# yf26/Hands-On-Point-Cloud-Processing

Measured on AMD Instinct MI355X. Metric: M correspondences/sec + ICP iter/sec, 120k-pt KITTI pair, 1/2/4/8 MI355X, higher is better.
Workload: dtype f32

## Files before the change

hands-on-point-cloud-processing_amd/__init__.py:

```python
from __future__ import annotations

import ctypes as C
import os
import weakref

import numpy as np

_HERE = os.path.dirname(os.path.abspath(__file__))
LIB_PATH = os.environ.get("PCR_LIB_PATH") or os.path.join(_HERE, "libpcr_hip.so")
INCLUDE_DIR = os.path.join(os.path.dirname(_HERE), "include")

PCR_SOA, PCR_AOS3, PCR_AOS4, PCR_AOS6 = 0, 1, 2, 6
PCR_FPS_F32, PCR_FPS_F64 = 0, 1
PCR_KMEANS_PY, PCR_KMEANS_CPP = 0, 1
PCR_EMPTY_CLUSTER = 1
PCR_SPECTRAL_DUPLICATE, PCR_SPECTRAL_COMPLEX, PCR_SPECTRAL_NOT_CONVERGED, PCR_SPECTRAL_FEW_SEEDS = 2, 3, 4, 5
ERRORS = {0: "ok", -1: "bad argument", -2: "HIP error", -3: "out of memory", -4: "bad state",
          -5: "RCCL/collective error", -6: "no correspondence kept"}

_lib = None


class PcrError(RuntimeError):
    pass
# ... 77 lines not shown
    _fields_ = [("kind", C.c_int32), ("reserved0", C.c_uint32), ("beta1", C.c_double), ("beta2", C.c_double), ("eps", C.c_double), ("weight_decay", C.c_double),
                ("momentum", C.c_double), ("dampening", C.c_double), ("reserved", C.c_double * 4)]


class OptimInfo(C.Structure):
    _fields_ = [("desc", OptimDesc), ("step", C.c_uint64), ("state_bytes", C.c_uint64), ("attached", C.c_uint32), ("n_ranges", C.c_uint32)]


OPTIM_ADAM, OPTIM_SGD = 1, 2

ALLREDUCE_FN = C.CFUNCTYPE(C.c_int, C.c_void_p, C.POINTER(C.c_double), C.c_int)

ABI_SYMBOLS = [
    "pcr_device_count", "pcr_ctx_create", "pcr_ctx_destroy", "pcr_ctx_sync", "pcr_ctx_last_error", "pcr_version", "pcr_ctx_device_info",
    "pcr_cloud_create", "pcr_cloud_clone", "pcr_cloud_assign", "pcr_cloud_read", "pcr_cloud_size", "pcr_cloud_destroy",
    "pcr_nn1_f32", "pcr_nn1_f32_async", "pcr_nn1_fetch", "pcr_transform_f32", "pcr_kabsch_sums", "pcr_kabsch_solve", "pcr_kabsch_grid_exponent", "pcr_kabsch_limbs_to_sums",
    "pcr_icp_p2p_f32", "pcr_icp_last_chain", "pcr_icp_last_snapshots", "pcr_icp_replica_members", "pcr_icp_move_route", "pcr_icp_solve_route", "pcr_icp_solve_in_search_auto", "pcr_s3_walk_visits", "pcr_plane_count_f64", "pcr_plane_mask_f64", "pcr_knn_f64", "pcr_radius_f64",
    "pcr_comm_unique_id", "pcr_comm_init_rccl", "pcr_comm_init_callback", "pcr_comm_destroy", "pcr_comm_selftest", "pcr_shard_range",
    "pcr_prof_reset", "pcr_prof_get", "pcr_prof_get_each", "pcr_tune_set",
    "pcr_grid_stats", "pcr_nn1_stats", "pcr_selftest_mfma_bf16", "pcr_selftest_mfma_f16", "pcr_selftest_mfma_bf16_v2", "pcr_selftest_mfma_f16_v2", "pcr_selftest_sign_f16", "pcr_selftest_sphere_f16", "pcr_ctx_mfma_check", "pcr_voxel_filter_f32", "pcr_iss_keypoints_f32", "pcr_icp_p2plane_f32", "pcr_cloud_knn_f64", "pcr_normals_knn_f64", "pcr_cloud_pca_f64", "pcr_fast_eigen3x3", "pcr_ground_seeds_f64", "pcr_ground_detection_f64",
    "pcr_nn1_desc_f32", "pcr_match_union_f32", "pcr_match_inter_f32", "pcr_ransac_sample_quads", "pcr_consensus_count_f32", "pcr_ransac_global_f32", "pcr_db64_create", "pcr_db64_destroy", "pcr_db64_size", "pcr_db64_knn", "pcr_db64_radius",
    "pcr_ctx_trim", "pcr_ctx_parked_bytes", "pcr_cloud_shard_spatial", "pcr_cloud_global_index", "pcr_cloud_sort_for_target", "pcr_nn1_f32_loop",
    "pcr_db64_radius_rows", "pcr_rows_destroy", "pcr_rows_info", "pcr_rows_row_ptr", "pcr_rows_fetch", "pcr_rows_reduce", "pcr_rows_moments",
    "pcr_dbscan_f32", "pcr_statistical_outlier_f32", "pcr_fpfh33_f32", "pcr_harris3d_f32", "pcr_voxel_grid_normals_f32", "pcr_normal_space_sample_f32",
    "pcr_fps_f32", "pcr_ball_query_f32", "pcr_group_points_f32", "pcr_objects_from_labels_f32", "pcr_points_in_boxes_f64", "pcr_label_aabb_f32",
    "pcr_pn2_model_create", "pcr_pn2_model_destroy", "pcr_pn2_model_info", "pcr_sa_mlp_max_f32", "pcr_pn2_forward_f32",
    "pcr_pn2_msg_model_create", "pcr_pn2_msg_model_info", "pcr_ball_query_multi_f32", "pcr_sa_msg_mlp_max_f32",
    "pcr_pn1_model_create", "pcr_pn1_model_info", "pcr_pointwise_chain_max_f32", "pcr_pointnet_forward_f32",
    "pcr_pn2_trainer_create", "pcr_pn2_trainer_destroy", "pcr_pn2_trainer_info", "pcr_pn2_trainer_set_weights", "pcr_pn2_trainer_get_weights", "pcr_pn2_train_grad_f32",
    "pcr_pn1_trainer_create", "pcr_pointnet_train_grad_f32",
    "pcr_pn2_msg_trainer_create", "pcr_pn2_msg_trainer_info",
# ... 32 lines not shown
    L.pcr_cloud_size.restype = sz
    L.pcr_cloud_size.argtypes = [vp]
    L.pcr_cloud_destroy.argtypes = [vp, vp]
    L.pcr_nn1_f32.argtypes = [vp, vp, vp, vp, vp]
    L.pcr_nn1_f32_async.argtypes = [vp, vp, vp]
    L.pcr_nn1_fetch.argtypes = [vp, sz, vp, vp]
    L.pcr_ctx_trim.argtypes = [vp]
    L.pcr_cloud_shard_spatial.argtypes = [vp, vp, vp, C.c_int, C.c_int, C.c_int, C.POINTER(vp)]
    L.pcr_cloud_global_index.argtypes = [vp, vp, vp]
    L.pcr_ctx_parked_bytes.argtypes = [vp, C.POINTER(C.c_uint64)]
    L.pcr_cloud_sort_for_target.argtypes = [vp, vp, vp, vp]
    L.pcr_nn1_f32_loop.argtypes = [vp, vp, vp, C.c_float]
    L.pcr_transform_f32.argtypes = [vp, vp, vp]
    L.pcr_kabsch_sums.argtypes = [vp, vp, vp, C.c_float, vp, C.POINTER(C.c_int64), C.POINTER(C.c_float)]
    L.pcr_kabsch_solve.argtypes = [vp, vp, vp]
    L.pcr_kabsch_grid_exponent.argtypes = [C.c_float, C.c_float]
    L.pcr_kabsch_limbs_to_sums.argtypes = [vp, C.c_int, vp]
    L.pcr_icp_p2p_f32.argtypes = [vp, vp, vp, vp, C.POINTER(IcpParams), vp, C.POINTER(IcpStats)]
    L.pcr_icp_last_chain.argtypes = [vp]
    L.pcr_icp_last_snapshots.argtypes = [vp]
    L.pcr_icp_replica_members.argtypes = [C.c_uint32, C.c_uint32]
    L.pcr_icp_replica_members.restype = C.c_uint32
    L.pcr_icp_move_route.argtypes = [C.c_uint64, C.c_uint64, C.c_int] + [C.c_int64] * 7
    L.pcr_icp_solve_route.argtypes = [C.c_uint64, C.c_uint64, C.c_int] + [C.c_int64] * 8
    L.pcr_icp_solve_in_search_auto.argtypes = []
    L.pcr_icp_solve_in_search_auto.restype = C.c_uint64
    L.pcr_s3_walk_visits.argtypes = [C.c_uint32, vp, vp, C.c_uint32, vp, sz, C.POINTER(sz)]
    L.pcr_plane_count_f64.argtypes = [vp, vp, vp, sz, C.c_double, vp]
    L.pcr_plane_mask_f64.argtypes = [vp, vp, vp, C.c_double, vp, C.POINTER(C.c_int64)]
    L.pcr_knn_f64.argtypes = [vp, vp, sz, vp, sz, C.c_int, vp, vp]
# ... 207 lines not shown


def spectral_select_k(eigenvalues) -> int:
    e = np.ascontiguousarray(eigenvalues, np.float64)
    return int(lib().pcr_spectral_select_k(e.ctypes.data, e.shape[0]))


def kabsch_solve(sums):
    s = np.ascontiguousarray(sums, np.float64)
    R = np.zeros(9, np.float32)
    t = np.zeros(3, np.float32)
    rc = lib().pcr_kabsch_solve(s.ctypes.data, R.ctypes.data, t.ctypes.data)
    return rc, R.reshape(3, 3), t


class Cloud:

    def __init__(self, ctx: "Context", handle):
        self.ctx = ctx
        self.h = handle
        ctx._handles.add(self)

    def __del__(self):
        try:
            self.free()
        except Exception:
            pass

    def __len__(self):
        return int(lib().pcr_cloud_size(self.h))
# ... 1325 lines not shown
                                             qd.ctypes.data, qd.shape[0], thr, R.ctypes.data, tv.ctypes.data, C.byref(best), C.byref(win),
                                             counts.ctypes.data))
        return win.value, R.reshape(3, 3), tv, best.value, counts[: qd.shape[0]]

    def transform(self, cloud: Cloud, T):
        T = np.ascontiguousarray(T, np.float32).reshape(16)
        self._ck(lib().pcr_transform_f32(self.h, cloud.h, T.ctypes.data))

    def kabsch_sums(self, tgt: Cloud, src: Cloud, max_corr: float):
        sums = np.zeros(16, np.float64)
        last = C.c_int64()
        d2 = C.c_float()
        self._ck(lib().pcr_kabsch_sums(self.h, tgt.h, src.h, max_corr, sums.ctypes.data, C.byref(last), C.byref(d2)))
        return sums, last.value, d2.value

    def icp_point2point(self, src: Cloud, tgt: Cloud, init_T=None, max_corr=1.0, max_iter=20, eps=1e-8):
        T0 = np.eye(4, dtype=np.float32) if init_T is None else np.ascontiguousarray(init_T, np.float32)
        out = np.zeros(16, np.float32)
        prm = IcpParams(max_corr, max_iter, eps)
        st = IcpStats()
        self._ck(lib().pcr_icp_p2p_f32(self.h, src.h, tgt.h, T0.ctypes.data, C.byref(prm), out.ctypes.data, C.byref(st)))
        stats = {f: getattr(st, f) for f, _ in IcpStats._fields_ if f != "reserved"}
        return out.reshape(4, 4), stats

    def icp_last_chain(self) -> int:
        return int(lib().pcr_icp_last_chain(self.h))

    def icp_last_snapshots(self) -> int:
        return int(lib().pcr_icp_last_snapshots(self.h))

# ... 74 lines not shown
```

hands-on-point-cloud-processing_amd/csrc/api.cpp:

```cpp
#include "pcr_internal.hpp"
#include "numerics.hpp"

#include <cmath>
#include <limits>
#include <new>

namespace pcr {

int fail(pcr_ctx* ctx, int code, const char* what, hipError_t e)
{
    if (ctx) {
        ctx->err = what ? what : "";
        if (e != hipSuccess) {
            ctx->err += ": ";
            ctx->err += hipGetErrorString(e);
        }
    }
    return code;
}

int ensure_keys(pcr_ctx* ctx, size_t n)
{
    if (n <= ctx->keys_cap) return PCR_OK;
    if (ctx->keys) PCR_HIP(ctx, hipFree(ctx->keys));
// ... 516 lines not shown

int pcr_kabsch_limbs_to_sums(double row[55], int e, double sums[16])
{
    if (!row || !sums) return PCR_ERR_ARG;
    num::limbs_normalize_row(row);
    num::limbs_to_sums(row, e, sums);
    return PCR_OK;
}

int pcr_kabsch_solve(const double sums[16], float R[9], float t[3])
{
    if (!sums || !R || !t) return PCR_ERR_ARG;
    return kabsch_solve(sums, R, t);
}

int pcr_prof_reset(pcr_ctx* ctx)
{
    if (!ctx) return PCR_ERR_ARG;
    PCR_HIP(ctx, hipStreamSynchronize(ctx->stream));
    prof_flush(ctx);
    ctx->prof.clear();
    return PCR_OK;
}

int pcr_prof_get(pcr_ctx* ctx, const char* kernel, uint64_t* launches, double* total_ms)
{
    if (!ctx || !kernel) return PCR_ERR_ARG;
    PCR_HIP(ctx, hipStreamSynchronize(ctx->stream));
    prof_flush(ctx);
    auto it = ctx->prof.find(kernel);
// ... 228 lines not shown
```

hands-on-point-cloud-processing_amd/csrc/icp_finish.hpp:

```cpp
#pragma once

#include "pcr_internal.hpp"
#include "numerics.hpp"

#include <cstddef>

#pragma clang fp contract(off)

namespace pcr {

constexpr int KB_NL = num::KB_NL;
constexpr int KB_ROW = 58;
constexpr int KB_NLC = 40;

__device__ __forceinline__ void row_to_out18(int k, const double (&row)[KB_ROW], int e, double* out)
{
    if (k < 6) out[k] = num::limbs_value(row + 3 * k, 2, e - 2 * num::KB_W);
    else if (k < 15) out[k] = num::limbs_value(row + 18 + 4 * (k - 6), 3, 2 * e - 3 * num::KB_W);
    else if (k == 15) out[15] = row[54];
    else if (k == 16) {
        const unsigned long long lk = (unsigned long long)__double_as_longlong(row[55]);
        out[16] = row[54] > 0.0 ? (double)(uint32_t)(lk >> 32) : -1.0;
        out[17] = row[54] > 0.0 ? (double)__uint_as_float((uint32_t)(lk & 0xFFFFFFFFull)) : 0.0;
        out[18] = row[56];
// ... 65 lines not shown
    } else if (k == 15) {
        row[54] = (double)s_acc[0][KB_NLC - 1];
    } else if (k == 16) {
        row[55] = __longlong_as_double(s_acc[0][KB_NLC + 1]);
        row[56] = s_acc[0][KB_NLC] != 0 ? 1.0 : 0.0;
        row[57] = 0.0;
    }
}

__device__ __forceinline__ void fin_wave_sync()
{
    __builtin_amdgcn_fence(__ATOMIC_ACQ_REL, "wavefront");
    __builtin_amdgcn_wave_barrier();
}

struct IcpFinishLds {
    long long acc[ACC_R][ACC_W];
    double row[KB_ROW];
    double o18[19];
    IcpState st;
#ifdef PCR_SV_PROF
    unsigned long long pt_replicas;
#endif
};

constexpr int FIN_ACC_PER_LANE = ACC_R * ACC_W / 64;
static_assert(ACC_R * ACC_W % 64 == 0, "a wave reads the replicas in whole rounds");
struct IcpFinishLoads {
    uint32_t stw;
    long long acc[FIN_ACC_PER_LANE];
// ... 17 lines not shown
        fin_wave_sync();
        return false;
    }
#pragma unroll
    for (int i = 0; i < FIN_ACC_PER_LANE; i++) (&F.acc[0][0])[l + 64 * i] = Q.acc[i];
    fin_wave_sync();
#ifdef PCR_SV_PROF
    if (l == 0) F.pt_replicas = __builtin_amdgcn_s_memrealtime();
#endif
    if (l < KB_NLC + 2) acc_fold_column(F.acc, l);
    fin_wave_sync();
    acc_to_row(F.acc, l, F.row);
    fin_wave_sync();
    row_to_out18(l, F.row, e, F.o18);
    fin_wave_sync();
    if (l == 0) icp_state_step(&F.st, F.o18, F.o18[16] >= 0.0, (float)F.o18[17], F.o18[18] != 0.0);
    fin_wave_sync();
    return true;
}

__device__ __forceinline__ void finish_publish(int l, bool stepped, const IcpFinishLds& F, IcpState* st_out, double* out, IcpSnapSlot* snap, unsigned long long seq)
{
    static_assert(offsetof(IcpSnapSlot, state) == 0, "a snapshot's words, and behind them its sequence number");
    if (stepped && l < 19) out[l] = F.o18[l];
    if (l < ST_WORDS) reinterpret_cast<uint32_t*>(st_out)[l] = reinterpret_cast<const uint32_t*>(&F.st)[l];
    if (!snap) return;
    if (l < ST_WORDS) reinterpret_cast<uint32_t*>(&snap->state)[l] = reinterpret_cast<const uint32_t*>(&F.st)[l];
    fin_wave_sync();
    if (l == 0) __hip_atomic_store(&snap->seq, seq, __ATOMIC_RELEASE, __HIP_MEMORY_SCOPE_SYSTEM);
}

}
// ... 1 lines not shown
```

hands-on-point-cloud-processing_amd/csrc/kabsch.hip:

```cpp
#include "grid_common.hpp"
#include "icp_finish.hpp"
#include "numerics.hpp"

#include <algorithm>
#include <cmath>
#include <cstddef>

#pragma clang fp contract(off)

namespace pcr {

constexpr int KB_BLOCK = 256;
constexpr int KB_NV = 16;
constexpr int KB_MAX_BLOCKS = 8192;
static_assert(KB_ROW * KB_MAX_BLOCKS == 8192 * 58, "api.cpp sizes ctx->partials as 8192 x 58 doubles");

__device__ __forceinline__ double wave_sum(double v)
{
#pragma unroll
    for (int off = 32; off > 0; off >>= 1) v += __shfl_down(v, off, 64);
    return v;
}

__device__ __forceinline__ unsigned long long wave_max_u64(unsigned long long v)
// ... 341 lines not shown

__global__ __launch_bounds__(KF_BLOCK) void icp_update_kernel(const double* __restrict__ partials, uint32_t n_blocks, int e, IcpState* st,
                                                              double* __restrict__ out)
{
    __shared__ double red[KF_GROUPS][64];
    __shared__ double row[KB_ROW];
    __shared__ double o18[19];
    __shared__ IcpState s_st;
    icp_state_stage(st, &s_st);
    if (s_st.stop) return;
    if (s_st.stop_after_transform) { if (threadIdx.x == 0) st->stop = 1; return; }
    reduce_rows(partials, n_blocks, red, row);
    row_to_out18(row, e, o18);
    __syncthreads();
    if (threadIdx.x < 19) out[threadIdx.x] = o18[threadIdx.x];
    if (threadIdx.x == 0) {
        icp_state_step(&s_st, o18, o18[16] >= 0.0, (float)o18[17], o18[18] != 0.0);
        *st = s_st;
    }
}

struct SeedArgs {
    const float* tx; const float* ty; const float* tz;
    unsigned long long* keys;
    uint32_t nt;
};

__device__ __forceinline__ void seed_next_search(const SeedArgs& sd, uint32_t i, uint32_t n, float x, float y, float z)
{
    if (i >= n) return;
    const uint32_t j = (uint32_t)(sd.keys[i] & 0xFFFFFFFFull);
    unsigned long long key = ~0ull;
    if (j < sd.nt) {
// ... 23 lines not shown
        for (int u = 0; u < 4; u++)
            if (4 * i + u < n) sk[u] = sd.keys[4 * i + u];
#pragma unroll
        for (int u = 0; u < 4; u++) {
            const uint32_t j = (uint32_t)(sk[u] & 0xFFFFFFFFull);
            if (j < sd.nt) { sq[u][0] = sd.tx[j]; sq[u][1] = sd.ty[j]; sq[u][2] = sd.tz[j]; }
        }
    }
    icp_state_stage(st_in, &s_st);
    const int phase = s_st.stop ? 0 : (s_st.stop_after_transform ? 1 : 2);
    if (phase == 2) {
        reduce_rows(partials, n_blocks, red, row);
        row_to_out18(row, e, o18);
        __syncthreads();
        if (blockIdx.x == 0 && threadIdx.x < 19) out[threadIdx.x] = o18[threadIdx.x];
        if (threadIdx.x == 0) icp_state_step(&s_st, o18, o18[16] >= 0.0, (float)o18[17], o18[18] != 0.0);
    } else if (phase == 1) {
        if (threadIdx.x == 0) s_st.stop = 1;
    }
    __syncthreads();
    if (blockIdx.x == 0 && threadIdx.x == 0) *st_out = s_st;
    if (s_st.stop || !mine) return;
    const float r0 = s_st.Rd[0], r1 = s_st.Rd[1], r2 = s_st.Rd[2], r3 = s_st.Rd[3], r4 = s_st.Rd[4], r5 = s_st.Rd[5],
                r6 = s_st.Rd[6], r7 = s_st.Rd[7], r8 = s_st.Rd[8], t0 = s_st.td[0], t1 = s_st.td[1], t2 = s_st.td[2];
    float4 ox, oy, oz;
#define PCR_ROW(o, a, b, c, tt)                      \
    o.x = ((a * px.x + b * py.x) + c * pz.x) + tt;   \
    o.y = ((a * px.y + b * py.y) + c * pz.y) + tt;   \
    o.z = ((a * px.z + b * py.z) + c * pz.z) + tt;   \
    o.w = ((a * px.w + b * py.w) + c * pz.w) + tt;
    PCR_ROW(ox, r0, r1, r2, t0)
// ... 146 lines not shown
                    const unsigned long long pt_c = __builtin_amdgcn_s_memrealtime();
                    atomicAdd(prof + 12, pt_c - pt_b); atomicMax(prof + 13, pt_c - pt_b); atomicAdd(prof + 14, 1ull); atomicAdd(prof + 15, pt_b - pt_a);
                }
#endif
            }
            s_tmo = tmo;
        }
    }
    __syncthreads();
    const bool tmo = s_tmo != 0;
    if (phase == 2 && !tmo) {
        reduce_rows(partials, gridDim.x, red, row);
        row_to_out18(row, plan.e, o18);
        __syncthreads();
        if (blockIdx.x == 0 && threadIdx.x < 19) out[threadIdx.x] = o18[threadIdx.x];
        if (threadIdx.x == 0) icp_state_step(&s_st, o18, o18[16] >= 0.0, (float)o18[17], o18[18] != 0.0);
    } else if (threadIdx.x == 0) {
        s_st.stop = 1;
        if (tmo) {
            s_st.barrier_timeout = 1;
            __hip_atomic_store(&st_out->barrier_timeout, 1, __ATOMIC_RELAXED, __HIP_MEMORY_SCOPE_AGENT);
        }
    }
    __syncthreads();
    if (blockIdx.x == 0 && threadIdx.x < ST_WORDS && (threadIdx.x != FS_TMO_WORD || s_st.barrier_timeout))
        reinterpret_cast<uint32_t*>(st_out)[threadIdx.x] = reinterpret_cast<const uint32_t*>(&s_st)[threadIdx.x];
    if (s_st.stop || !mine) return;
    const float r0 = s_st.Rd[0], r1 = s_st.Rd[1], r2 = s_st.Rd[2], r3 = s_st.Rd[3], r4 = s_st.Rd[4], r5 = s_st.Rd[5],
                r6 = s_st.Rd[6], r7 = s_st.Rd[7], r8 = s_st.Rd[8], t0 = s_st.td[0], t1 = s_st.td[1], t2 = s_st.td[2];
    float4 ox, oy, oz;
#define PCR_ROW(o, a, b, c, tt)                      \
// ... 239 lines not shown
        __syncthreads();
#ifdef PCR_SS_PROF
        const unsigned long long pt_c2 = __builtin_amdgcn_s_memrealtime();
#endif
        const int k = threadIdx.x;
        if (k < KB_NLC + 2) acc_fold_column(s_acc, k);
        __syncthreads();
        acc_to_row(s_acc, k, row);
        __syncthreads();
#ifdef PCR_SS_PROF
        unsigned long long pt_d = __builtin_amdgcn_s_memrealtime(), pt_e = pt_d;
#endif
        row_to_out18(row, plan.e, o18);
        __syncthreads();
        if (threadIdx.x < 19) out[threadIdx.x] = o18[threadIdx.x];
        if (threadIdx.x == 0) {
            icp_state_step(&s_st, o18, o18[16] >= 0.0, (float)o18[17], o18[18] != 0.0);
#ifdef PCR_SS_PROF
            pt_e = __builtin_amdgcn_s_memrealtime();
#endif
        }
        __syncthreads();
        if (threadIdx.x < ST_WORDS) reinterpret_cast<uint32_t*>(st_out)[threadIdx.x] = reinterpret_cast<const uint32_t*>(&s_st)[threadIdx.x];
#ifdef PCR_SS_PROF
        asm volatile("s_waitcnt vmcnt(0)" ::: "memory");
        const unsigned long long pt_f = __builtin_amdgcn_s_memrealtime();
#endif
        ss_snapshot(snap, seq, &s_st);
#ifdef PCR_SS_PROF
        asm volatile("s_waitcnt vmcnt(0)" ::: "memory");
        if (prof && threadIdx.x == 0) {
            prof[0] = pt_d - pt_c; prof[1] = pt_e - pt_d; prof[11] = pt_f - pt_e; prof[4] = snap ? __builtin_amdgcn_s_memrealtime() - pt_f : 0ull;
// ... 96 lines not shown
}

__global__ __launch_bounds__(64) void icp_update_from_sums_kernel(double* __restrict__ buf, int nranks, int e, IcpState* st)
{
    __shared__ double row[KB_NL + 1];
    __shared__ double sums[16];
    __shared__ IcpState s_st;
    const int k = threadIdx.x;
    if (k < KB_NL) row[k] = buf[k];
    icp_state_stage(st, &s_st);
    if (s_st.stop) return;
    if (k < 6) { num::limbs_normalize(row + 3 * k, 2); sums[k] = num::limbs_value(row + 3 * k, 2, e - 2 * num::KB_W); }
    else if (k < 15) { num::limbs_normalize(row + 18 + 4 * (k - 6), 3); sums[k] = num::limbs_value(row + 18 + 4 * (k - 6), 3, 2 * e - 3 * num::KB_W); }
    else if (k == 15) sums[15] = row[54];
    __syncthreads();
    if (k != 0) return;
    const int ls = icp_last_slot(buf, nranks);
    const bool any = ls >= 0;
    const float d2 = any ? (float)buf[57 + 2 * ls] : 0.0f;
    icp_state_step(&s_st, sums, any, d2, buf[55] != 0.0);
    *st = s_st;
}

__global__ __launch_bounds__(256) void transform_state_kernel(float* __restrict__ x, float* __restrict__ y,
                                                              float* __restrict__ z, uint32_t n, uint32_t n4, IcpState* st, SeedArgs sd)
{
    const uint32_t i = blockIdx.x * blockDim.x + threadIdx.x;
    if (i >= n4) return;
    float4 px = reinterpret_cast<float4*>(x)[i];
    float4 py = reinterpret_cast<float4*>(y)[i];
    float4 pz = reinterpret_cast<float4*>(z)[i];
    const float r0 = st->Rd[0], r1 = st->Rd[1], r2 = st->Rd[2], r3 = st->Rd[3], r4 = st->Rd[4], r5 = st->Rd[5],
                r6 = st->Rd[6], r7 = st->Rd[7], r8 = st->Rd[8], t0 = st->td[0], t1 = st->td[1], t2 = st->td[2];
    const int stop = st->stop;
    if (stop) return;
    float4 ox, oy, oz;
// ... 198 lines not shown
        hipLaunchKernelGGL(icp_finish_kernel, dim3(1), dim3(64), 0, ctx->stream, ctx->icp_acc_dev + (size_t)set * ICP_ACC_REPLICAS * ICP_ACC_WORDS, plan.e,
                           st_in, st_out, ctx->dev_out, snap, seq);
    }
    PCR_HIP(ctx, hipGetLastError());
    return PCR_OK;
}

int launch_icp_reduce_slots(pcr_ctx* ctx, uint32_t n_blocks, int nranks, int rank, bool have_points, const uint32_t* gidx)
{
    hipLaunchKernelGGL(icp_reduce_slots_kernel, dim3(1), dim3(KF_BLOCK), 0, ctx->stream, ctx->partials, n_blocks, ctx->dev_out, nranks, rank,
                       have_points ? 1 : 0, gidx);
    PCR_HIP(ctx, hipGetLastError());
    return PCR_OK;
}

int launch_icp_update_from_sums(pcr_ctx* ctx, int nranks, IcpState* st_dev, const KabschPlan& plan)
{
    hipLaunchKernelGGL(icp_update_from_sums_kernel, dim3(1), dim3(64), 0, ctx->stream, ctx->dev_out, nranks, plan.e, st_dev);
    PCR_HIP(ctx, hipGetLastError());
    return PCR_OK;
}

int launch_transform_state(pcr_ctx* ctx, pcr_cloud* c, IcpState* st_dev, const pcr_cloud* seed_tgt)
{
    if (c->n) {
        const uint32_t n4 = (uint32_t)((c->n + 3) / 4);
        const SeedArgs sd = seed_args(ctx, c, seed_tgt);
        ProfScope p(ctx, "transform");
        hipLaunchKernelGGL(transform_state_kernel, dim3((n4 + 255) / 256), dim3(256), 0, ctx->stream, c->x(), c->y(), c->z(),
                           (uint32_t)c->n, n4, st_dev, sd);
// ... 111 lines not shown
```

hands-on-point-cloud-processing_amd/csrc/numerics.cpp:

```cpp
#include "pcr_internal.hpp"
#include "numerics.hpp"

#include <cmath>

namespace pcr {

void svd3(const double A[9], double U[9], double S[3], double V[9]) { num::svd3(A, U, S, V); }

int kabsch_solve(const double sums[16], float R[9], float t[3])
{
    return num::kabsch_solve(sums, R, t) == 0 ? PCR_OK : PCR_ERR_EMPTY;
}

void mat4_mul_f32(const float A[16], const float B[16], float out[16]) { num::mat4_mul_f32(A, B, out); }

}

namespace pcr {
namespace {

constexpr int EIG_MAX = 16;
constexpr int EIG_DENSE_MAX = 32;

template <int MAX>
struct EigWork {
    int n, low, high, perm[MAX];
// ... 388 lines not shown
```

hands-on-point-cloud-processing_amd/csrc/pcr_internal.hpp:

```cpp
#pragma once

#include <hip/hip_runtime.h>

#include <cstdint>
#include <cstdio>
#include <cstring>
#include <map>
#include <memory>
#include <string>
#include <vector>

#include "pcr.h"
#include "scratch_layout.hpp"

namespace pcr {

constexpr size_t PAD = 1024;
constexpr int PCR_NSTATS = 16;
constexpr int ICP_ACC_REPLICAS = 8, ICP_ACC_WORDS = 48;
constexpr int ICP_ACC_SETS = 2;
__host__ __device__ constexpr uint32_t icp_replica_members(uint32_t blocks, uint32_t r)
{
    return r < (uint32_t)ICP_ACC_REPLICAS && r < blocks ? (blocks - r + ICP_ACC_REPLICAS - 1) / ICP_ACC_REPLICAS : 0u;
}
// ... 298 lines not shown
int ball_query_device(pcr_ctx* ctx, const float* x, const float* y, const float* z, const float* qx, const float* qy, const float* qz, const uint32_t* seg_dev,
                      const uint32_t* centre_seg_dev, size_t nq, double radius, size_t nsample, uint32_t* idx_dev, uint32_t* cnt_dev);
int ball_query_multi_device(pcr_ctx* ctx, const float* x, const float* y, const float* z, const float* qx, const float* qy, const float* qz, const uint32_t* seg_dev,
                            const uint32_t* centre_seg_dev, size_t nq, size_t n_radii, const double* radii, const uint32_t* nsamples, uint32_t* const* idx_dev,
                            uint32_t* const* cnt_dev);
inline unsigned long long splitmix_key(unsigned long long seed, unsigned long long a)
{
    unsigned long long zz = seed ^ (0x9E3779B97F4A7C15ull * (a + 1ull));
    zz = (zz ^ (zz >> 30)) * 0xBF58476D1CE4E5B9ull;
    zz = (zz ^ (zz >> 27)) * 0x94D049BB133111EBull;
    return zz ^ (zz >> 31);
}

void svd3(const double A[9], double U[9], double S[3], double V[9]);
int kabsch_solve(const double sums[16], float R[9], float t[3]);
void mat4_mul_f32(const float A[16], const float B[16], float out[16]);
int eig_small(int n, const double* a, double* wr, double* wi, double* vec);
int eig_dense(int n, const double* a, double* wr, double* wi, double* vec);
int spectral_select_k(const double* eig, int n_eig);
const double* mat64_rows_dev(const pcr_mat64* m);

int comm_allreduce_f64(pcr_ctx* ctx, double* host_buf, double* dev_buf, int n);
__host__ __device__ inline int icp_last_slot(const double* buf, int nranks)
{
    int best = -1;
    double key = 0.5;
    for (int r = 0; r < nranks; r++)
        if (buf[56 + 2 * r] > key) { key = buf[56 + 2 * r]; best = r; }
    return best;
}
// ... 3 lines not shown
```

include/pcr.h:

```cpp
#ifndef PCR_H
#define PCR_H

#include <stddef.h>
#include <stdint.h>

#ifdef __cplusplus
extern "C" {
#endif

#define PCR_OK 0
#define PCR_ERR_ARG (-1)
#define PCR_ERR_HIP (-2)
#define PCR_ERR_NOMEM (-3)
#define PCR_ERR_STATE (-4)
#define PCR_ERR_COMM (-5)
#define PCR_ERR_EMPTY (-6)

typedef struct pcr_ctx pcr_ctx;
typedef struct pcr_cloud pcr_cloud;

enum pcr_layout {
    PCR_SOA = 0,
    PCR_AOS3 = 1,
    PCR_AOS4 = 2,
// ... 16 lines not shown
int pcr_cloud_destroy(pcr_ctx* ctx, pcr_cloud* c);
int pcr_ctx_trim(pcr_ctx* ctx);
int pcr_ctx_parked_bytes(const pcr_ctx* ctx, uint64_t* bytes);

int pcr_nn1_f32(pcr_ctx* ctx, const pcr_cloud* tgt, const pcr_cloud* src, uint32_t* idx, float* d2);
int pcr_nn1_f32_async(pcr_ctx* ctx, const pcr_cloud* tgt, const pcr_cloud* src);
int pcr_cloud_sort_for_target(pcr_ctx* ctx, const pcr_cloud* tgt, pcr_cloud* cloud, uint32_t* orig_index);
int pcr_nn1_f32_loop(pcr_ctx* ctx, const pcr_cloud* tgt, const pcr_cloud* src, float max_corr);
int pcr_nn1_fetch(pcr_ctx* ctx, size_t n, uint32_t* idx, float* d2);

int pcr_transform_f32(pcr_ctx* ctx, pcr_cloud* cloud, const float T[16]);

int pcr_kabsch_sums(pcr_ctx* ctx, const pcr_cloud* tgt, const pcr_cloud* src, float max_corr,
                    double sums[16], int64_t* last_kept, float* last_d2);
int pcr_kabsch_solve(const double sums[16], float R[9], float t[3]);

typedef struct {
    float max_corr;
    uint64_t max_iter;
    float eps;
} pcr_icp_params;

typedef struct {
    uint64_t iters_run;
    int32_t converged;
    int32_t empty_pairs;
    uint64_t last_pairs;
    float last_loss;
    float reserved;
    double ms_total;
// ... 369 lines not shown
```

Baseline: 3384.

## Solve Kabsch SVD and pose update across wave lanes instead of lane 0

```diff
diff --git a/hands-on-point-cloud-processing_amd/__init__.py b/hands-on-point-cloud-processing_amd/__init__.py
--- a/hands-on-point-cloud-processing_amd/__init__.py
+++ b/hands-on-point-cloud-processing_amd/__init__.py
@@ -115,7 +115,7 @@
 ABI_SYMBOLS = [
     "pcr_device_count", "pcr_ctx_create", "pcr_ctx_destroy", "pcr_ctx_sync", "pcr_ctx_last_error", "pcr_version", "pcr_ctx_device_info",
     "pcr_cloud_create", "pcr_cloud_clone", "pcr_cloud_assign", "pcr_cloud_read", "pcr_cloud_size", "pcr_cloud_destroy",
-    "pcr_nn1_f32", "pcr_nn1_f32_async", "pcr_nn1_fetch", "pcr_transform_f32", "pcr_kabsch_sums", "pcr_kabsch_solve", "pcr_kabsch_grid_exponent", "pcr_kabsch_limbs_to_sums",
+    "pcr_nn1_f32", "pcr_nn1_f32_async", "pcr_nn1_fetch", "pcr_transform_f32", "pcr_kabsch_sums", "pcr_kabsch_solve", "pcr_kabsch_solve_lanes", "pcr_kabsch_solve_batch_device", "pcr_kabsch_grid_exponent", "pcr_kabsch_limbs_to_sums",
     "pcr_icp_p2p_f32", "pcr_icp_last_chain", "pcr_icp_last_snapshots", "pcr_icp_replica_members", "pcr_icp_move_route", "pcr_icp_solve_route", "pcr_icp_solve_in_search_auto", "pcr_s3_walk_visits", "pcr_plane_count_f64", "pcr_plane_mask_f64", "pcr_knn_f64", "pcr_radius_f64",
     "pcr_comm_unique_id", "pcr_comm_init_rccl", "pcr_comm_init_callback", "pcr_comm_destroy", "pcr_comm_selftest", "pcr_shard_range",
     "pcr_prof_reset", "pcr_prof_get", "pcr_prof_get_each", "pcr_tune_set",
@@ -178,6 +178,8 @@
     L.pcr_transform_f32.argtypes = [vp, vp, vp]
     L.pcr_kabsch_sums.argtypes = [vp, vp, vp, C.c_float, vp, C.POINTER(C.c_int64), C.POINTER(C.c_float)]
     L.pcr_kabsch_solve.argtypes = [vp, vp, vp]
+    L.pcr_kabsch_solve_lanes.argtypes = [vp, vp, vp]
+    L.pcr_kabsch_solve_batch_device.argtypes = [vp, vp, sz, vp, vp, vp]
     L.pcr_kabsch_grid_exponent.argtypes = [C.c_float, C.c_float]
     L.pcr_kabsch_limbs_to_sums.argtypes = [vp, C.c_int, vp]
     L.pcr_icp_p2p_f32.argtypes = [vp, vp, vp, vp, C.POINTER(IcpParams), vp, C.POINTER(IcpStats)]
@@ -415,6 +417,14 @@
     return rc, R.reshape(3, 3), t
 
 
+def kabsch_solve_lanes(sums):
+    s = np.ascontiguousarray(sums, np.float64)
+    R = np.zeros(9, np.float32)
+    t = np.zeros(3, np.float32)
+    rc = lib().pcr_kabsch_solve_lanes(s.ctypes.data, R.ctypes.data, t.ctypes.data)
+    return rc, R.reshape(3, 3), t
+
+
 class Cloud:
 
     def __init__(self, ctx: "Context", handle):
@@ -1770,6 +1780,13 @@
         self._ck(lib().pcr_kabsch_sums(self.h, tgt.h, src.h, max_corr, sums.ctypes.data, C.byref(last), C.byref(d2)))
         return sums, last.value, d2.value
 
+    def kabsch_solve_batch_device(self, sums):
+        s = np.ascontiguousarray(sums, np.float64).reshape(-1, 16)
+        n = s.shape[0]
+        R, t, rc = np.zeros((n, 9), np.float32), np.zeros((n, 3), np.float32), np.zeros(n, np.int32)
+        self._ck(lib().pcr_kabsch_solve_batch_device(self.h, s.ctypes.data, n, R.ctypes.data, t.ctypes.data, rc.ctypes.data))
+        return rc, R.reshape(n, 3, 3), t
+
     def icp_point2point(self, src: Cloud, tgt: Cloud, init_T=None, max_corr=1.0, max_iter=20, eps=1e-8):
         T0 = np.eye(4, dtype=np.float32) if init_T is None else np.ascontiguousarray(init_T, np.float32)
         out = np.zeros(16, np.float32)
diff --git a/hands-on-point-cloud-processing_amd/csrc/api.cpp b/hands-on-point-cloud-processing_amd/csrc/api.cpp
--- a/hands-on-point-cloud-processing_amd/csrc/api.cpp
+++ b/hands-on-point-cloud-processing_amd/csrc/api.cpp
@@ -554,6 +554,18 @@
     return kabsch_solve(sums, R, t);
 }
 
+int pcr_kabsch_solve_lanes(const double sums[16], float R[9], float t[3])
+{
+    if (!sums || !R || !t) return PCR_ERR_ARG;
+    return kabsch_solve_lanes(sums, R, t);
+}
+
+int pcr_kabsch_solve_batch_device(pcr_ctx* ctx, const double* sums, size_t n, float* R, float* t, int* rc)
+{
+    if (!ctx || (n && (!sums || !R || !t || !rc))) return fail(ctx, PCR_ERR_ARG, "pcr_kabsch_solve_batch_device");
+    return kabsch_solve_batch_device(ctx, sums, n, R, t, rc);
+}
+
 int pcr_prof_reset(pcr_ctx* ctx)
 {
     if (!ctx) return PCR_ERR_ARG;
diff --git a/hands-on-point-cloud-processing_amd/csrc/icp_finish.hpp b/hands-on-point-cloud-processing_amd/csrc/icp_finish.hpp
--- a/hands-on-point-cloud-processing_amd/csrc/icp_finish.hpp
+++ b/hands-on-point-cloud-processing_amd/csrc/icp_finish.hpp
@@ -2,6 +2,7 @@
 
 #include "pcr_internal.hpp"
 #include "numerics.hpp"
+#include "kabsch_wave.hpp"
 
 #include <cstddef>
 
@@ -103,6 +104,50 @@
     __builtin_amdgcn_wave_barrier();
 }
 
+__device__ __forceinline__ void icp_state_step_wave(int l, IcpState* st, const double* sums16, bool any_kept, float last_d2, bool overflow)
+{
+#ifdef PCR_SOLVE_SCALAR
+    if (l == 0) icp_state_step(st, sums16, any_kept, last_d2, overflow);
+    fin_wave_sync();
+#else
+    const int stop = st->stop, after = st->stop_after_transform;
+    const float last_loss = st->last_loss, eps = st->eps, T_mine = st->T_total[l & 15];
+    unsigned long long unchanged = st->unchanged;
+    const unsigned long long iters_run = st->iters_run, max_iter = st->max_iter;
+    fin_wave_sync();
+    if (!__builtin_amdgcn_readfirstlane(stop)) {
+        if (__builtin_amdgcn_readfirstlane(after)) { if (l == 0) st->stop = 1; }
+        else if (__builtin_amdgcn_readfirstlane((int)overflow)) { if (l == 0) { st->overflow = 1; st->stop = 1; } }
+        else {
+            float loss = 0.0f;
+            if (any_kept) loss = last_d2 * last_d2;
+            if (fabsf(last_loss - loss) < eps) unchanged++;
+            const bool converged = __builtin_amdgcn_readfirstlane((int)(unchanged > 15)) != 0;
+            if (l == 0) {
+                st->last_pairs = (unsigned long long)sums16[15];
+                st->loss = loss;
+                st->unchanged = unchanged;
+                if (converged) { st->converged = 1; st->stop = 1; }
+                else st->last_loss = loss;
+            }
+            if (!converged) {
+                const num::WaveLanes g{ l };
+                float R = 0.0f, t = 0.0f;
+                if (num::kabsch_solve_lanes(g, sums16, R, t) != 0) { if (l == 0) { st->empty = 1; st->stop = 1; } }
+                else {
+                    const float T_new = num::pose_compose_lanes(g, R, t, T_mine);
+                    if (l < 9) st->Rd[l] = R;
+                    if (l < 3) st->td[l] = t;
+                    if (l < 16) st->T_total[l] = T_new;
+                    if (l == 0) { st->iters_run = iters_run + 1; if (iters_run + 1 >= max_iter) st->stop_after_transform = 1; }
+                }
+            }
+        }
+    }
+    fin_wave_sync();
+#endif
+}
+
 struct IcpFinishLds {
     long long acc[ACC_R][ACC_W];
     double row[KB_ROW];
@@ -150,8 +195,7 @@
     fin_wave_sync();
     row_to_out18(l, F.row, e, F.o18);
     fin_wave_sync();
-    if (l == 0) icp_state_step(&F.st, F.o18, F.o18[16] >= 0.0, (float)F.o18[17], F.o18[18] != 0.0);
-    fin_wave_sync();
+    icp_state_step_wave(l, &F.st, F.o18, F.o18[16] >= 0.0, (float)F.o18[17], F.o18[18] != 0.0);
     return true;
 }
 
diff --git a/hands-on-point-cloud-processing_amd/csrc/kabsch.hip b/hands-on-point-cloud-processing_amd/csrc/kabsch.hip
--- a/hands-on-point-cloud-processing_amd/csrc/kabsch.hip
+++ b/hands-on-point-cloud-processing_amd/csrc/kabsch.hip
@@ -379,9 +379,9 @@
     row_to_out18(row, e, o18);
     __syncthreads();
     if (threadIdx.x < 19) out[threadIdx.x] = o18[threadIdx.x];
-    if (threadIdx.x == 0) {
-        icp_state_step(&s_st, o18, o18[16] >= 0.0, (float)o18[17], o18[18] != 0.0);
-        *st = s_st;
+    if (threadIdx.x < 64) {
+        icp_state_step_wave((int)threadIdx.x, &s_st, o18, o18[16] >= 0.0, (float)o18[17], o18[18] != 0.0);
+        if (threadIdx.x == 0) *st = s_st;
     }
 }
 
@@ -435,7 +435,7 @@
         row_to_out18(row, e, o18);
         __syncthreads();
         if (blockIdx.x == 0 && threadIdx.x < 19) out[threadIdx.x] = o18[threadIdx.x];
-        if (threadIdx.x == 0) icp_state_step(&s_st, o18, o18[16] >= 0.0, (float)o18[17], o18[18] != 0.0);
+        if (threadIdx.x < 64) icp_state_step_wave((int)threadIdx.x, &s_st, o18, o18[16] >= 0.0, (float)o18[17], o18[18] != 0.0);
     } else if (phase == 1) {
         if (threadIdx.x == 0) s_st.stop = 1;
     }
@@ -612,7 +612,7 @@
         row_to_out18(row, plan.e, o18);
         __syncthreads();
         if (blockIdx.x == 0 && threadIdx.x < 19) out[threadIdx.x] = o18[threadIdx.x];
-        if (threadIdx.x == 0) icp_state_step(&s_st, o18, o18[16] >= 0.0, (float)o18[17], o18[18] != 0.0);
+        if (threadIdx.x < 64) icp_state_step_wave((int)threadIdx.x, &s_st, o18, o18[16] >= 0.0, (float)o18[17], o18[18] != 0.0);
     } else if (threadIdx.x == 0) {
         s_st.stop = 1;
         if (tmo) {
@@ -882,8 +882,8 @@
         row_to_out18(row, plan.e, o18);
         __syncthreads();
         if (threadIdx.x < 19) out[threadIdx.x] = o18[threadIdx.x];
-        if (threadIdx.x == 0) {
-            icp_state_step(&s_st, o18, o18[16] >= 0.0, (float)o18[17], o18[18] != 0.0);
+        if (threadIdx.x < 64) {
+            icp_state_step_wave((int)threadIdx.x, &s_st, o18, o18[16] >= 0.0, (float)o18[17], o18[18] != 0.0);
 #ifdef PCR_SS_PROF
             pt_e = __builtin_amdgcn_s_memrealtime();
 #endif
@@ -1010,12 +1010,11 @@
     else if (k < 15) { num::limbs_normalize(row + 18 + 4 * (k - 6), 3); sums[k] = num::limbs_value(row + 18 + 4 * (k - 6), 3, 2 * e - 3 * num::KB_W); }
     else if (k == 15) sums[15] = row[54];
     __syncthreads();
-    if (k != 0) return;
     const int ls = icp_last_slot(buf, nranks);
     const bool any = ls >= 0;
     const float d2 = any ? (float)buf[57 + 2 * ls] : 0.0f;
-    icp_state_step(&s_st, sums, any, d2, buf[55] != 0.0);
-    *st = s_st;
+    icp_state_step_wave(k, &s_st, sums, any, d2, buf[55] != 0.0);
+    if (k == 0) *st = s_st;
 }
 
 __global__ __launch_bounds__(256) void transform_state_kernel(float* __restrict__ x, float* __restrict__ y,
@@ -1244,6 +1243,50 @@
     return PCR_OK;
 }
 
+constexpr int KSB_WAVES = 4;
+__global__ __launch_bounds__(64 * KSB_WAVES) void kabsch_solve_batch_kernel(const double* __restrict__ sums, uint32_t n, float* __restrict__ R, float* __restrict__ t,
+                                                                            int* __restrict__ rc)
+{
+    const int l = threadIdx.x & 63;
+    const uint32_t p = blockIdx.x * KSB_WAVES + (threadIdx.x >> 6);
+    if (p >= n) return;
+    const num::WaveLanes g{ l };
+    float Rl = 0.0f, tl = 0.0f;
+    const int r = num::kabsch_solve_lanes(g, sums + 16 * (size_t)p, Rl, tl);
+    if (l == 0) rc[p] = r == 0 ? PCR_OK : PCR_ERR_EMPTY;
+    if (r != 0) return;
+    if (l < 9) R[9 * (size_t)p + l] = Rl;
+    if (l < 3) t[3 * (size_t)p + l] = tl;
+}
+
+int kabsch_solve_batch_device(pcr_ctx* ctx, const double* sums, size_t n, float* R, float* t, int* rc)
+{
+    if (n == 0) return PCR_OK;
+    if (n > 0x7FFFFFFFull / 16) return fail(ctx, PCR_ERR_ARG, "pcr_kabsch_solve_batch_device: too many problems");
+    const size_t b_sums = n * 16 * sizeof(double), b_R = n * 9 * sizeof(float), b_t = n * 3 * sizeof(float), b_rc = n * sizeof(int);
+    char* dev = nullptr;
+    PCR_HIP(ctx, hipMalloc(reinterpret_cast<void**>(&dev), b_sums + b_R + b_t + b_rc));
+    double* d_sums = reinterpret_cast<double*>(dev);
+    float* d_R = reinterpret_cast<float*>(dev + b_sums);
+    float* d_t = reinterpret_cast<float*>(dev + b_sums + b_R);
+    int* d_rc = reinterpret_cast<int*>(dev + b_sums + b_R + b_t);
+    hipError_t e = hipMemcpyAsync(d_sums, sums, b_sums, hipMemcpyHostToDevice, ctx->stream);
+    if (e == hipSuccess) e = hipMemsetAsync(d_R, 0, b_R + b_t + b_rc, ctx->stream);
+    if (e == hipSuccess) {
+        hipLaunchKernelGGL(kabsch_solve_batch_kernel, dim3((uint32_t)((n + KSB_WAVES - 1) / KSB_WAVES)), dim3(64 * KSB_WAVES), 0, ctx->stream, d_sums, (uint32_t)n,
+                           d_R, d_t, d_rc);
+        e = hipGetLastError();
+    }
+    if (e == hipSuccess) e = hipMemcpyAsync(R, d_R, b_R, hipMemcpyDeviceToHost, ctx->stream);
+    if (e == hipSuccess) e = hipMemcpyAsync(t, d_t, b_t, hipMemcpyDeviceToHost, ctx->stream);
+    if (e == hipSuccess) e = hipMemcpyAsync(rc, d_rc, b_rc, hipMemcpyDeviceToHost, ctx->stream);
+    const hipError_t es = hipStreamSynchronize(ctx->stream);
+    if (e == hipSuccess) e = es;
+    (void)hipFree(dev);
+    if (e != hipSuccess) return fail(ctx, PCR_ERR_HIP, "pcr_kabsch_solve_batch_device", e);
+    return PCR_OK;
+}
+
 int launch_icp_update_from_sums(pcr_ctx* ctx, int nranks, IcpState* st_dev, const KabschPlan& plan)
 {
     hipLaunchKernelGGL(icp_update_from_sums_kernel, dim3(1), dim3(64), 0, ctx->stream, ctx->dev_out, nranks, plan.e, st_dev);
diff --git a/hands-on-point-cloud-processing_amd/csrc/kabsch_wave.hpp b/hands-on-point-cloud-processing_amd/csrc/kabsch_wave.hpp
--- /dev/null
+++ b/hands-on-point-cloud-processing_amd/csrc/kabsch_wave.hpp
@@ -0,0 +1,231 @@
+#pragma once
+
+#include "numerics.hpp"
+
+#pragma clang fp contract(off)
+
+namespace pcr {
+namespace num {
+
+template <class T, int N>
+struct LaneVec {
+    T v[N];
+    LaneVec() = default;
+    LaneVec(T s) { for (int i = 0; i < N; i++) v[i] = s; }
+};
+#define PCR_LV_BIN(OP, RT)                                                                                                                                \
+    template <class T, int N> inline LaneVec<RT, N> operator OP(const LaneVec<T, N>& a, const LaneVec<T, N>& b) { LaneVec<RT, N> r; for (int i = 0; i < N; i++) r.v[i] = a.v[i] OP b.v[i]; return r; } \
+    template <class T, int N> inline LaneVec<RT, N> operator OP(const LaneVec<T, N>& a, T b) { LaneVec<RT, N> r; for (int i = 0; i < N; i++) r.v[i] = a.v[i] OP b; return r; }                     \
+    template <class T, int N> inline LaneVec<RT, N> operator OP(T a, const LaneVec<T, N>& b) { LaneVec<RT, N> r; for (int i = 0; i < N; i++) r.v[i] = a OP b.v[i]; return r; }
+PCR_LV_BIN(+, T) PCR_LV_BIN(-, T) PCR_LV_BIN(*, T) PCR_LV_BIN(/, T) PCR_LV_BIN(&, T)
+PCR_LV_BIN(<, bool) PCR_LV_BIN(<=, bool) PCR_LV_BIN(>, bool) PCR_LV_BIN(>=, bool) PCR_LV_BIN(==, bool)
+#undef PCR_LV_BIN
+template <class T, int N> inline LaneVec<T, N> operator-(const LaneVec<T, N>& a) { LaneVec<T, N> r; for (int i = 0; i < N; i++) r.v[i] = -a.v[i]; return r; }
+using ::sqrt;
+template <int N> inline LaneVec<double, N> sqrt(const LaneVec<double, N>& a) { LaneVec<double, N> r; for (int i = 0; i < N; i++) r.v[i] = ::sqrt(a.v[i]); return r; }
+
+template <int N>
+struct HostLanes {
+    using D = LaneVec<double, N>; using F = LaneVec<float, N>; using I = LaneVec<int, N>; using B = LaneVec<bool, N>;
+    I lane() const { I r; for (int i = 0; i < N; i++) r.v[i] = i; return r; }
+    template <class T> LaneVec<T, N> get(const LaneVec<T, N>& v, int k) const { return LaneVec<T, N>(v.v[k]); }
+    template <class T> LaneVec<T, N> pick(const LaneVec<T, N>& v, const I& k) const { LaneVec<T, N> r; for (int i = 0; i < N; i++) r.v[i] = v.v[k.v[i] % N]; return r; }
+    mutable bool split = false;
+    bool uniform(const B& b) const
+    {
+        for (int i = 1; i < N; i++) if (b.v[i] != b.v[0]) split = true;
+        return b.v[0];
+    }
+    template <class T> LaneVec<T, N> sel(const B& c, const LaneVec<T, N>& a, const LaneVec<T, N>& b) const { LaneVec<T, N> r; for (int i = 0; i < N; i++) r.v[i] = c.v[i] ? a.v[i] : b.v[i]; return r; }
+    F to_f32(const D& a) const { F r; for (int i = 0; i < N; i++) r.v[i] = (float)a.v[i]; return r; }
+    D to_f64(const F& a) const { D r; for (int i = 0; i < N; i++) r.v[i] = (double)a.v[i]; return r; }
+    D ld(const double* p, const I& k) const { D r; for (int i = 0; i < N; i++) r.v[i] = p[k.v[i]]; return r; }
+};
+
+#if defined(__HIPCC__)
+struct WaveLanes {
+    using D = double; using F = float; using I = int; using B = bool;
+    int l;
+    __device__ __forceinline__ I lane() const { return l; }
+    __device__ __forceinline__ D get(D v, int k) const
+    {
+        const long long b = __double_as_longlong(v);
+        const uint32_t lo = (uint32_t)__builtin_amdgcn_readlane((int)(uint32_t)(b & 0xFFFFFFFFll), k), hi = (uint32_t)__builtin_amdgcn_readlane((int)(uint32_t)((unsigned long long)b >> 32), k);
+        return __longlong_as_double((long long)(((unsigned long long)hi << 32) | lo));
+    }
+    __device__ __forceinline__ D pick(D v, I k) const
+    {
+        const long long b = __double_as_longlong(v);
+        const uint32_t lo = (uint32_t)__builtin_amdgcn_ds_bpermute(k << 2, (int)(uint32_t)(b & 0xFFFFFFFFll)), hi = (uint32_t)__builtin_amdgcn_ds_bpermute(k << 2, (int)(uint32_t)((unsigned long long)b >> 32));
+        return __longlong_as_double((long long)(((unsigned long long)hi << 32) | lo));
+    }
+    __device__ __forceinline__ F pick(F v, I k) const { return __int_as_float(__builtin_amdgcn_ds_bpermute(k << 2, __float_as_int(v))); }
+    __device__ __forceinline__ bool uniform(B b) const { return __builtin_amdgcn_readfirstlane((int)b) != 0; }
+    __device__ __forceinline__ D sel(B c, D a, D b) const { return c ? a : b; }
+    __device__ __forceinline__ F sel(B c, F a, F b) const { return c ? a : b; }
+    __device__ __forceinline__ I sel(B c, I a, I b) const { return c ? a : b; }
+    __device__ __forceinline__ F to_f32(D a) const { return (float)a; }
+    __device__ __forceinline__ D to_f64(F a) const { return (double)a; }
+    __device__ __forceinline__ D ld(const double* p, I k) const { return p[k]; }
+};
+#endif
+
+template <class G>
+PCR_HD typename G::D lanes_abs(const G& g, const typename G::D& v) { return g.sel(v < 0.0, -v, v); }
+
+template <class G>
+PCR_HD typename G::D rows_sum3(const G& g, const typename G::D& p) { return (g.get(p, 0) + g.get(p, 1)) + g.get(p, 2); }
+
+template <int P, int Q, class G>
+PCR_HD bool jacobi_pair_lanes(const G& g, typename G::D (&x)[3])
+{
+    using D = typename G::D;
+    const double eps = 2.220446049250313e-16;
+    const D alpha = rows_sum3(g, x[P] * x[P]), beta = rows_sum3(g, x[Q] * x[Q]), gamma = rows_sum3(g, x[P] * x[Q]);
+    if (g.uniform(gamma == 0.0)) return false;
+    if (g.uniform(lanes_abs(g, gamma) <= eps * sqrt(alpha * beta))) return false;
+    const D zeta = (beta - alpha) / (2.0 * gamma);
+    const D tn = g.sel(zeta >= 0.0, D(1.0), D(-1.0)) / (lanes_abs(g, zeta) + sqrt(1.0 + zeta * zeta));
+    const D c = 1.0 / sqrt(1.0 + tn * tn), s = c * tn;
+    const D mp = x[P], mq = x[Q];
+    x[P] = c * mp - s * mq;
+    x[Q] = s * mp + c * mq;
+    return true;
+}
+
+template <int A, int B, class G>
+PCR_HD void order_cols_lanes(const G& g, typename G::D (&sv)[3], typename G::D (&x)[3])
+{
+    using D = typename G::D;
+    const typename G::B sw = sv[B] > sv[A];
+    const D sa = sv[A], sb = sv[B], xa = x[A], xb = x[B];
+    sv[A] = g.sel(sw, sb, sa); sv[B] = g.sel(sw, sa, sb);
+    x[A] = g.sel(sw, xb, xa); x[B] = g.sel(sw, xa, xb);
+}
+
+template <class G>
+PCR_HD void svd3_repair_lanes(const G& g, typename G::D (&U)[9], const bool (&have)[3])
+{
+    using D = typename G::D; using I = typename G::I; using B = typename G::B;
+    if (!have[0]) {
+        for (int r = 0; r < 3; r++)
+            for (int c = 0; c < 3; c++) U[3 * r + c] = D(r == c ? 1.0 : 0.0);
+        return;
+    }
+    if (!have[1]) {
+        const D u0[3] = { U[0], U[3], U[6] };
+        I k = I(0);
+        D uk = u0[0];
+        const B b1 = lanes_abs(g, u0[1]) < lanes_abs(g, uk);
+        k = g.sel(b1, I(1), k); uk = g.sel(b1, u0[1], uk);
+        const B b2 = lanes_abs(g, u0[2]) < lanes_abs(g, uk);
+        k = g.sel(b2, I(2), k); uk = g.sel(b2, u0[2], uk);
+        D v[3] = { -uk * u0[0], -uk * u0[1], -uk * u0[2] };
+        for (int i = 0; i < 3; i++) v[i] = g.sel(k == i, v[i] + 1.0, v[i]);
+        const D nv = sqrt(v[0] * v[0] + v[1] * v[1] + v[2] * v[2]);
+        U[1] = v[0] / nv; U[4] = v[1] / nv; U[7] = v[2] / nv;
+    }
+    if (!have[2]) {
+        U[2] = U[3] * U[7] - U[6] * U[4];
+        U[5] = U[6] * U[1] - U[0] * U[7];
+        U[8] = U[0] * U[4] - U[3] * U[1];
+    }
+}
+
+template <class G, class T>
+PCR_HD T lanes_of3(const G& g, const typename G::I& k, const T& a0, const T& a1, const T& a2) { return g.sel(k == 0, a0, g.sel(k == 1, a1, a2)); }
+
+template <class G>
+PCR_HD int kabsch_solve_lanes(const G& g, const double* sums, typename G::F& R_out, typename G::F& t_out)
+{
+    using D = typename G::D; using F = typename G::F; using I = typename G::I;
+    const double eps = 2.220446049250313e-16;
+    const I l = g.lane();
+    const D M = g.ld(sums, I(15));
+    if (!g.uniform(M > 0.0)) return -1;
+    const D mean = g.ld(sums, g.sel(l < 6, l, I(5))) / M;
+    const D pbar[3] = { g.get(mean, 0), g.get(mean, 1), g.get(mean, 2) }, qbar[3] = { g.get(mean, 3), g.get(mean, 4), g.get(mean, 5) };
+    const I i9 = g.sel(l < 9, l, I(8)), r9 = i9 / 3, c9 = i9 - 3 * r9;
+    const D h = g.ld(sums, 6 + i9) - M * lanes_of3(g, r9, qbar[0], qbar[1], qbar[2]) * lanes_of3(g, c9, pbar[0], pbar[1], pbar[2]);
+    const I rw = g.sel(l < 3, l, I(0)), rr = l - 3;
+    D x[3];
+    for (int c = 0; c < 3; c++) x[c] = g.sel(l < 3, g.pick(h, 3 * rw + c), g.sel(rr == c, D(1.0), D(0.0)));
+    for (int sweep = 0; sweep < 60; sweep++) {
+        const bool r01 = jacobi_pair_lanes<0, 1>(g, x);
+        const bool r02 = jacobi_pair_lanes<0, 2>(g, x);
+        const bool r12 = jacobi_pair_lanes<1, 2>(g, x);
+        if (!(r01 || r02 || r12)) break;
+    }
+    const D d0 = rows_sum3(g, x[0] * x[0]), d1 = rows_sum3(g, x[1] * x[1]), d2 = rows_sum3(g, x[2] * x[2]);
+    const D root = sqrt(lanes_of3(g, l, d0, d1, d2));
+    D sv[3] = { g.get(root, 0), g.get(root, 1), g.get(root, 2) };
+    order_cols_lanes<0, 1>(g, sv, x);
+    order_cols_lanes<0, 2>(g, sv, x);
+    order_cols_lanes<1, 2>(g, sv, x);
+    const D smax = sv[0];
+    bool have[3];
+    for (int c = 0; c < 3; c++) have[c] = g.uniform((sv[c] > 0.0) & (sv[c] > smax * eps * 8.0));
+    const D w9 = lanes_of3(g, c9, g.pick(x[0], r9), g.pick(x[1], r9), g.pick(x[2], r9)), sv9 = lanes_of3(g, c9, sv[0], sv[1], sv[2]);
+    D u9 = g.sel((sv9 > 0.0) & (sv9 > smax * eps * 8.0), w9 / sv9, D(0.0));
+    if (!(have[0] && have[1] && have[2])) {
+        D U[9];
+        for (int k = 0; k < 9; k++) U[k] = g.get(u9, k);
+        svd3_repair_lanes(g, U, have);
+        u9 = U[8];
+        for (int k = 7; k >= 0; k--) u9 = g.sel(i9 == k, U[k], u9);
+    }
+    D rd9;
+    {
+        const D u0 = g.pick(u9, 3 * r9), u1 = g.pick(u9, 3 * r9 + 1), u2 = g.pick(u9, 3 * r9 + 2);
+        const D v0 = g.pick(x[0], 3 + c9), v1 = g.pick(x[1], 3 + c9), v2 = g.pick(x[2], 3 + c9);
+        rd9 = u0 * v0 + u1 * v1 + u2 * v2;
+    }
+    D Rd[9];
+    for (int k = 0; k < 9; k++) Rd[k] = g.get(rd9, k);
+    const D det = Rd[0] * (Rd[4] * Rd[8] - Rd[5] * Rd[7]) - Rd[1] * (Rd[3] * Rd[8] - Rd[5] * Rd[6])
+                + Rd[2] * (Rd[3] * Rd[7] - Rd[4] * Rd[6]);
+    if (g.uniform(det < 0.0)) {
+        const D v0 = g.pick(x[0], 3 + r9), v1 = g.pick(x[1], 3 + r9), v2 = g.pick(x[2], 3 + r9) * det;
+        const D u0 = g.pick(u9, 3 * c9), u1 = g.pick(u9, 3 * c9 + 1), u2 = g.pick(u9, 3 * c9 + 2);
+        rd9 = v0 * u0 + v1 * u1 + v2 * u2;
+    }
+    const F Rf = g.to_f32(rd9);
+    const I r3 = g.sel(l < 3, l, I(2));
+    const D Rp = (g.to_f64(g.pick(Rf, 3 * r3)) * pbar[0] + g.to_f64(g.pick(Rf, 3 * r3 + 1)) * pbar[1]) + g.to_f64(g.pick(Rf, 3 * r3 + 2)) * pbar[2];
+    R_out = Rf;
+    t_out = g.to_f32(lanes_of3(g, r3, qbar[0], qbar[1], qbar[2]) - Rp);
+    return 0;
+}
+
+template <class G>
+PCR_HD typename G::F pose_compose_lanes(const G& g, const typename G::F& R, const typename G::F& t, const typename G::F& T_total)
+{
+    using F = typename G::F; using I = typename G::I; using B = typename G::B;
+    const I l = g.lane();
+    const I i16 = g.sel(l < 16, l, I(15)), r4 = i16 / 4, c4 = i16 - 4 * r4;
+    const B top = r4 < 3;
+    const I rr = g.sel(top, r4, I(0));
+    const F a0 = g.sel(top, g.pick(R, 3 * rr), F(0.0f)), a1 = g.sel(top, g.pick(R, 3 * rr + 1), F(0.0f)), a2 = g.sel(top, g.pick(R, 3 * rr + 2), F(0.0f)),
+            a3 = g.sel(top, g.pick(t, rr), F(1.0f));
+    F acc = a0 * g.pick(T_total, c4);
+    acc = acc + a1 * g.pick(T_total, 4 + c4);
+    acc = acc + a2 * g.pick(T_total, 8 + c4);
+    acc = acc + a3 * g.pick(T_total, 12 + c4);
+    return acc;
+}
+
+inline int kabsch_solve_host_lanes(const double sums[16], float R[9], float t[3])
+{
+    using G = HostLanes<16>;
+    const G g;
+    G::F Rl(0.0f), tl(0.0f);
+    const int rc = kabsch_solve_lanes(g, sums, Rl, tl);
+    if (g.split) return -2;
+    if (rc != 0) return rc;
+    for (int k = 0; k < 9; k++) R[k] = Rl.v[k];
+    for (int k = 0; k < 3; k++) t[k] = tl.v[k];
+    return 0;
+}
+
+}
+}
diff --git a/hands-on-point-cloud-processing_amd/csrc/numerics.cpp b/hands-on-point-cloud-processing_amd/csrc/numerics.cpp
--- a/hands-on-point-cloud-processing_amd/csrc/numerics.cpp
+++ b/hands-on-point-cloud-processing_amd/csrc/numerics.cpp
@@ -1,5 +1,6 @@
 #include "pcr_internal.hpp"
 #include "numerics.hpp"
+#include "kabsch_wave.hpp"
 
 #include <cmath>
 
@@ -10,6 +11,12 @@
 int kabsch_solve(const double sums[16], float R[9], float t[3])
 {
     return num::kabsch_solve(sums, R, t) == 0 ? PCR_OK : PCR_ERR_EMPTY;
+}
+
+int kabsch_solve_lanes(const double sums[16], float R[9], float t[3])
+{
+    const int rc = num::kabsch_solve_host_lanes(sums, R, t);
+    return rc == 0 ? PCR_OK : rc == -1 ? PCR_ERR_EMPTY : PCR_ERR_STATE;
 }
 
 void mat4_mul_f32(const float A[16], const float B[16], float out[16]) { num::mat4_mul_f32(A, B, out); }
diff --git a/hands-on-point-cloud-processing_amd/csrc/pcr_internal.hpp b/hands-on-point-cloud-processing_amd/csrc/pcr_internal.hpp
--- a/hands-on-point-cloud-processing_amd/csrc/pcr_internal.hpp
+++ b/hands-on-point-cloud-processing_amd/csrc/pcr_internal.hpp
@@ -336,6 +336,8 @@
 
 void svd3(const double A[9], double U[9], double S[3], double V[9]);
 int kabsch_solve(const double sums[16], float R[9], float t[3]);
+int kabsch_solve_lanes(const double sums[16], float R[9], float t[3]);
+int kabsch_solve_batch_device(pcr_ctx* ctx, const double* sums, size_t n, float* R, float* t, int* rc);
 void mat4_mul_f32(const float A[16], const float B[16], float out[16]);
 int eig_small(int n, const double* a, double* wr, double* wi, double* vec);
 int eig_dense(int n, const double* a, double* wr, double* wi, double* vec);
diff --git a/include/pcr.h b/include/pcr.h
--- a/include/pcr.h
+++ b/include/pcr.h
@@ -54,6 +54,8 @@
 int pcr_kabsch_sums(pcr_ctx* ctx, const pcr_cloud* tgt, const pcr_cloud* src, float max_corr,
                     double sums[16], int64_t* last_kept, float* last_d2);
 int pcr_kabsch_solve(const double sums[16], float R[9], float t[3]);
+int pcr_kabsch_solve_lanes(const double sums[16], float R[9], float t[3]);
+int pcr_kabsch_solve_batch_device(pcr_ctx* ctx, const double* sums, size_t n, float* R, float* t, int* rc);
 
 typedef struct {
     float max_corr;
```

New measurement: 3660 (median of 6 runs). 8.1% higher.
